# tohtsky/myFM

Hardware: AMD Instinct MI355X
Metric: Gibbs iterations/sec (rank=32) (higher is better)
Workload: dtype f64

## Files before the change

myfm_amd/csrc/mfm_res.hpp:

```cpp
#pragma once
#include <algorithm>
#include <cstdlib>
#include <cstring>
#include <atomic>
#include <string>
#include <thread>
#include <vector>

#include "mfm_common.hpp"
#include "mfm_mf_kernels.hpp"

namespace mfm {

#ifndef MFM_RES_CH
#define MFM_RES_CH 4
#endif
constexpr int RES_MAX_PEERS = 8;

struct ResArgs {
  double2 *eq;
  const double *e_in;
  double *e_slots;
  const int32_t *perm;
  const uint32_t *uidw;
// ... 48 lines not shown
  __hip_atomic_store(p + 1, b, __ATOMIC_RELAXED, __HIP_MEMORY_SCOPE_AGENT);
}

enum { RES_BAR_START = 0, RES_BAR_TOP = 16, RES_BAR_XCNT = 32, RES_BAR_GEN = 160, RES_BAR_CENSUS = 288, RES_BAR_WORDS = 416 };
struct ResBar {
  int xcc;
  unsigned long long n_x, nx;
};

__device__ __forceinline__ bool res_spin(const ResArgs &a, const unsigned long long *w, unsigned long long target, bool &dead) {
  unsigned spins = 0;
  while (__hip_atomic_load(w, __ATOMIC_RELAXED, __HIP_MEMORY_SCOPE_AGENT) < target) {
#ifndef MFM_RES_NO_SLEEP
    __builtin_amdgcn_s_sleep(1);
#endif
    if ((++spins & 1023u) == 0u) {
      if (spins > (1u << 22) || __hip_atomic_load(a.error, __ATOMIC_RELAXED, __HIP_MEMORY_SCOPE_AGENT) != 0) {
        __hip_atomic_store(a.error, 1, __ATOMIC_RELAXED, __HIP_MEMORY_SCOPE_AGENT);
        dead = true;
        return false;
      }
    }
  }
  return true;
}

__device__ __forceinline__ bool res_spin_sys(const ResArgs &a, const unsigned long long *w, unsigned long long target, bool &dead) {
  unsigned spins = 0;
  while (__hip_atomic_load(w, __ATOMIC_RELAXED, __HIP_MEMORY_SCOPE_SYSTEM) < target) {
    __builtin_amdgcn_s_sleep(2);
    if ((++spins & 1023u) == 0u) {
      const int seen = __hip_atomic_load(a.error, __ATOMIC_RELAXED, __HIP_MEMORY_SCOPE_AGENT);
      if (spins > (1u << 23) || seen != 0) {
        if (seen == 0) __hip_atomic_store(a.error, 2, __ATOMIC_RELAXED, __HIP_MEMORY_SCOPE_AGENT);
        dead = true;
        return false;
      }
    }
  }
  return true;
}

__device__ __forceinline__ void res_bar_init(const ResArgs &a, ResBar &rb, bool &dead) {
  unsigned x;
  asm volatile("s_getreg_b32 %0, hwreg(HW_REG_XCC_ID, 0, 4)" : "=s"(x));
  rb.xcc = (int)(x & 7u);
  __hip_atomic_fetch_add(a.bar + RES_BAR_CENSUS + 16 * rb.xcc, 1ull, __ATOMIC_RELAXED, __HIP_MEMORY_SCOPE_AGENT);
  asm volatile("s_waitcnt vmcnt(0)" ::: "memory");
  __hip_atomic_fetch_add(a.bar + RES_BAR_START, 1ull, __ATOMIC_RELAXED, __HIP_MEMORY_SCOPE_AGENT);
  rb.n_x = 1;
  rb.nx = 1;
  if (!res_spin(a, a.bar + RES_BAR_START, (unsigned long long)a.n_wg, dead)) return;
  rb.nx = 0;
  for (int i = 0; i < 8; i++) {
    const unsigned long long c = __hip_atomic_load(a.bar + RES_BAR_CENSUS + 16 * i, __ATOMIC_RELAXED, __HIP_MEMORY_SCOPE_AGENT);
    rb.nx += c > 0 ? 1 : 0;
    if (i == rb.xcc) rb.n_x = c;
  }
}

__device__ __forceinline__ void res_grid_barrier(const ResArgs &a, const ResBar &rb, unsigned long long k, int tid, bool &dead) {
  asm volatile("s_waitcnt vmcnt(0)" ::: "memory");
  __syncthreads();
  if (tid == 0 && !dead) {
    const unsigned long long old =
        __hip_atomic_fetch_add(a.bar + RES_BAR_XCNT + 16 * rb.xcc, 1ull, __ATOMIC_RELAXED, __HIP_MEMORY_SCOPE_AGENT);
    if (old + 1 == k * rb.n_x) {
      __builtin_amdgcn_fence(__ATOMIC_RELEASE, "agent");
      asm volatile("s_waitcnt vmcnt(0)" ::: "memory");
      __hip_atomic_fetch_add(a.bar + RES_BAR_TOP, 1ull, __ATOMIC_RELAXED, __HIP_MEMORY_SCOPE_AGENT);
      if (res_spin(a, a.bar + RES_BAR_TOP, k * rb.nx, dead))
        __hip_atomic_store(a.bar + RES_BAR_GEN + 16 * rb.xcc, k, __ATOMIC_RELAXED, __HIP_MEMORY_SCOPE_AGENT);
    } else {
      res_spin(a, a.bar + RES_BAR_GEN + 16 * rb.xcc, k, dead);
    }
    __builtin_amdgcn_fence(__ATOMIC_ACQUIRE, "agent");
  }
  __syncthreads();
}

typedef double res_d16_t __attribute__((ext_vector_type(16)));
typedef unsigned res_u4_t __attribute__((ext_vector_type(4)));

template <int NT, int NGV, int NGL, bool XCH = false, bool OVF = false>
__global__ __launch_bounds__(NT) void k_mf_resident(ResArgs a) {
  extern __shared__ __attribute__((aligned(16))) char res_smem[];
  constexpr int NW = NT / WAVE, NG = NGV + NGL, R = 16 * NG, RL = 16 * NGL;
  constexpr int B = 4;
  const int g = (int)blockIdx.x, tid = threadIdx.x, lane = tid & 63;
  const int wv = __builtin_amdgcn_readfirstlane(tid >> 6);
  const int U = a.umax;
  const double alpha_k = a.scal ? a.scal[0] : a.alpha, e_shift_k = a.scal ? a.scal[2] : a.e_shift;
  const int ngx = OVF ? a.ngx : 0, NGt = NG + ngx, Rt = 16 * NGt;
  d2_t *utab = (d2_t *)res_smem;
  double *elds = (double *)(utab + U);
  double *acc1 = elds + (size_t)RL * NT;
  double *acc2 = acc1 + NW * U;
  d2_t *wcarry = (d2_t *)(acc2 + NW * U);
  int *wflag = (int *)(wcarry + NW);
  const int32_t *perm_g = a.perm + (int64_t)g * Rt * NT;
  const int u0 = a.wg_user_ptr[g], nu = a.wg_user_ptr[g + 1] - u0;
  const int rb0 = a.wg_run_ptr[g];
  const int pad_item = a.n_items;
  const unsigned rb0b = 4u * (unsigned)rb0, padb = 16u * (unsigned)pad_item;
  const char *run_item_b = (const char *)a.run_item, *dv_b = (const char *)a.dv;
  double *acc1w = acc1 + wv * U, *acc2w = acc2 + wv * U;
  bool dead = false;
  unsigned long long nbar = 0;
  ResBar rbar;
  rbar.xcc = 0;
  rbar.n_x = rbar.nx = 1;
#define RES_STAMP0(k) \
  if (a.prof && tid == 0) a.prof[(int64_t)g * a.n_sw * 64 + 56 + (k)] = __builtin_amdgcn_s_memrealtime()
  RES_STAMP0(0);
  if (tid == 0) res_bar_init(a, rbar, dead);
  RES_STAMP0(1);
  const int wv_hi = wv >> 2;
#define RES_PRIO(j)                  \
  if ((((j) & 1) ^ wv_hi) != 0)      \
    __builtin_amdgcn_s_setprio(1);   \
  else                               \
    __builtin_amdgcn_s_setprio(0)
  const int trash_run = a.wg_run_ptr[g] + a.wg_nruns[g];
#define RES_STAMP(k)                                                                                      \
  if (a.prof && tid == 0) a.prof[((int64_t)g * a.n_sw + (f - f_first)) * 64 + (k)] = __builtin_amdgcn_s_memrealtime()

  for (int i = tid; i < 2 * NW * U; i += NT) acc1[i] = 0.0;
  for (int i = tid; i < U; i += NT) utab[i] = d2_t{0.0, 0.0};

  res_u4_t uw[NG];
  unsigned ux[NG];
  unsigned hbv[NG], nbv[NG];
#pragma unroll
  for (int j = 0; j < NG; j++) {
#pragma unroll
    for (int w = 0; w < 4; w++) uw[j][w] = a.uidw[((int64_t)g * (5 * NGt) + 5 * j + w) * NT + tid];
    ux[j] = a.uidw[((int64_t)g * (5 * NGt) + 5 * j + 4) * NT + tid];
    hbv[j] = a.headw[((int64_t)g * NGt + j) * NT + tid];
    nbv[j] = hbv[j] | (j == 0 ? 1u : 0u);
  }
  const unsigned nbx0 = OVF && ngx > 0 ? a.headw[((int64_t)g * NGt + NG) * NT + tid] : 0u;
  double *eog = OVF ? a.e_slots + ((int64_t)g * Rt + 16 * NG) * NT + tid : nullptr;
  const uint32_t *uidw_x = a.uidw + ((int64_t)g * (5 * NGt) + 5 * NG) * NT + tid;
  const uint32_t *headw_x = a.headw + ((int64_t)g * NGt + NG) * NT + tid;
  const int run0 = a.first_run[g * NT + tid];
  const bool head0 = (hbv[0] & 1u) != 0u;
#define RES_NIB(j, q) ((((nbv[j]) | ((j) + 1 < NG ? nbv[(j) + 1 < NG ? (j) + 1 : (j)] << 16 : nbx0 << 16)) >> (4 * (q))) & 15u)
#define RES_UIDS(j, bb, uid)                                                     \
  {                                                                              \
    const unsigned lo_ = uw[j][bb];                                              \
    uid[0] = (int)(lo_ & 0x3ffu);                                                \
    uid[1] = (int)((lo_ >> 10) & 0x3ffu);                                        \
    uid[2] = (int)((lo_ >> 20) & 0x3ffu);                                        \
    uid[3] = (int)((lo_ >> 30) | (((ux[j] >> (8 * (bb))) & 0xffu) << 2));        \
  }

#define RES_UIDSX(bb, uid)                                                       \
  {                                                                              \
    const unsigned lo_ = uwx[bb];                                                \
    uid[0] = (int)(lo_ & 0x3ffu);                                                \
    uid[1] = (int)((lo_ >> 10) & 0x3ffu);                                        \
    uid[2] = (int)((lo_ >> 20) & 0x3ffu);                                        \
    uid[3] = (int)((lo_ >> 30) | (((uxx >> (8 * (bb))) & 0xffu) << 2));          \
  }

#define RES_OPAQUE()                                                                            \
  _Pragma("unroll") for (int j_ = 0; j_ < NG; j_++) {                                           \
    asm volatile("" : "+v"(uw[j_]), "+v"(ux[j_]), "+v"(hbv[j_]), "+v"(nbv[j_]));                \
  }
  res_d16_t ev[NGV > 0 ? NGV : 1];
#pragma unroll
  for (int j = 0; j < NG; j++) {
#pragma unroll 1
    for (int bb = 0; bb < 4; bb++) {
      int row[B];
#pragma unroll
      for (int k = 0; k < B; k++) row[k] = a.e_in ? 0 : perm_g[(16 * j + 4 * bb + k) * NT + tid];
#pragma unroll
      for (int k = 0; k < B; k++) {
        const double x = (a.e_in ? a.e_in[((int64_t)g * Rt + 16 * j + 4 * bb + k) * NT + tid] : a.eq[row[k] < 0 ? 0 : row[k]].x) + e_shift_k;
        if (j < NGV)
          ev[j < NGV ? j : 0][4 * bb + k] = x;
        else
          elds[(16 * (j - NGV) + 4 * bb + k) * NT + tid] = x;
      }
    }
  }
  if (OVF) {
    for (int jx = 0; jx < ngx; jx++) {
#pragma unroll 4
      for (int i = 0; i < 16; i++) {
        const int64_t sl = 16 * (NG + jx) + i;
        const int row = a.e_in ? 0 : perm_g[sl * NT + tid];
        const double x = (a.e_in ? a.e_in[((int64_t)g * Rt + sl) * NT + tid] : a.eq[row < 0 ? 0 : row].x) + e_shift_k;
        eog[(16 * jx + i) * NT] = x;
      }
    }
  }
  __syncthreads();

  RES_STAMP0(2);
  const int f_first = a.f_begin - a.linear;
  for (int f = f_first; f < a.f_end; f++) {
    const bool lin = f < a.f_begin;
    double *Vf = lin ? a.w : a.V + (int64_t)f * a.D;
    const double *zf = lin ? a.zw : a.z + (int64_t)(f - a.f_begin) * a.D;
    const double *lamf = lin ? a.lam_w : a.lam + (int64_t)f * a.n_groups;
    const double *muf = lin ? a.mu_w : a.mu + (int64_t)f * a.n_groups;
    int uj = 0;
    double uold = 0.0, uz = 0.0, ulam = 0.0, umu = 0.0;
    if (tid < nu) {
      const int2 d = a.user_desc[u0 + tid];
      uj = d.x;
      uold = Vf[uj];
      uz = zf[uj];
      ulam = lamf[d.y];
      umu = muf[d.y];
    }
    RES_STAMP(0);
    {
      RES_OPAQUE();
      asm volatile(";; res sweep A");
      unsigned rcb = 4u * (unsigned)(run0 - 1);
      int itA[B];
      d2_t ddA[B];
      {
        int it0[B];
        const unsigned n0 = RES_NIB(0, 0), n1 = RES_NIB(0, 1);
#pragma unroll
        for (int k = 0; k < B; k++) {
          rcb += ((n0 >> k) & 1u) << 2;
          it0[k] = *(const int *)(run_item_b + ((n0 >> k) & 1u ? rcb : rb0b));
        }
#pragma unroll
        for (int k = 0; k < B; k++) {
          rcb += ((n1 >> k) & 1u) << 2;
          itA[k] = *(const int *)(run_item_b + ((n1 >> k) & 1u ? rcb : rb0b));
        }
#pragma unroll
        for (int k = 0; k < B; k++) ddA[k] = *(const d2_t *)(dv_b + ((n0 >> k) & 1u ? (unsigned)it0[k] << 4 : padb));
      }
      d2_t ddc = d2_t{0.0, 0.0};
      int itB[B];
      d2_t ddB[B];
#define RES_STEP_A(j, bb, iti, ito, ddi, ddo)                                                                              \
  {                                                                                                                        \
    const unsigned n4 = RES_NIB(j, bb), n4a = RES_NIB(j, (bb) + 1), n4b = RES_NIB(j, (bb) + 2);                            \
    _Pragma("unroll") for (int k = 0; k < B; k++) {                                                                        \
      rcb += ((n4b >> k) & 1u) << 2;                                                                                       \
      ito[k] = *(const int *)(run_item_b + ((n4b >> k) & 1u ? rcb : rb0b));                                                \
    }                                                                                                                      \
// ... 25 lines not shown
    const unsigned n4 = ((nbw >> (4 * (bb))) & 15u), n4a = ((nbw >> (4 * ((bb) + 1))) & 15u), n4b = ((nbw >> (4 * ((bb) + 2))) & 15u);                            \
    _Pragma("unroll") for (int k = 0; k < B; k++) {                                                                        \
      rcb += ((n4b >> k) & 1u) << 2;                                                                                       \
      ito[k] = *(const int *)(run_item_b + ((n4b >> k) & 1u ? rcb : rb0b));                                                \
    }                                                                                                                      \
    _Pragma("unroll") for (int k = 0; k < B; k++)                                                                          \
      ddo[k] = *(const d2_t *)(dv_b + ((n4a >> k) & 1u ? (unsigned)iti[k] << 4 : padb));                                   \
    int uid[B];                                                                                                            \
    RES_UIDSX(bb, uid);                                                                                                      \
    double up[B], ex[B];                                                                                                   \
    _Pragma("unroll") for (int k = 0; k < B; k++) {                                                                        \
      up[k] = utab[uid[k]][0];                                                                                             \
      ex[k] = eo[4 * (bb) + k];              \
    }                                                                                                                      \
    _Pragma("unroll") for (int k = 0; k < B; k++) {                                                                        \
      const bool need = ((n4 >> k) & 1u) != 0u;                                                                            \
      ddc[0] = need ? ddi[k][0] : ddc[0];                                                                                  \
      ddc[1] = need ? ddi[k][1] : ddc[1];                                                                                  \
      const double er = ex[k] + up[k] * ddc[0];                                                                            \
      eo[4 * (bb) + k] = er;                                                             \
      const double c = ddc[1];                                                                                             \
      __hip_atomic_fetch_add(&acc1w[uid[k]], (-er) * c, __ATOMIC_RELAXED, __HIP_MEMORY_SCOPE_WORKGROUP);                   \
      __hip_atomic_fetch_add(&acc2w[uid[k]], c * c, __ATOMIC_RELAXED, __HIP_MEMORY_SCOPE_WORKGROUP);                       \
    }                                                                                                                      \
  }
#pragma unroll
      for (int j = 0; j < NG; j++) {
        RES_PRIO(j);
#pragma unroll
        for (int bp = 0; bp < 2; bp++) {
          RES_STEP_A(j, 2 * bp, itA, itB, ddA, ddB);
          RES_STEP_A(j, 2 * bp + 1, itB, itA, ddB, ddA);
        }
      }
      asm volatile(";; res sweep end");
      if (OVF) {
        unsigned hb_c = nbx0;
        for (int jx = 0; jx < ngx; jx++) {
          res_u4_t uwx;
#pragma unroll
          for (int w = 0; w < 4; w++) uwx[w] = uidw_x[(5 * jx + w) * NT];
          const unsigned uxx = uidw_x[(5 * jx + 4) * NT];
          const unsigned hb_n = jx + 1 < ngx ? headw_x[(jx + 1) * NT] : 0u;
          const unsigned nbw = hb_c | (hb_n << 16);
          res_d16_t eo;
#pragma unroll
          for (int i = 0; i < 16; i++) eo[i] = eog[(16 * jx + i) * NT];
#pragma unroll 1
          for (int bp = 0; bp < 2; bp++) {
            RES_STEP_AX(2 * bp, itA, itB, ddA, ddB);
            RES_STEP_AX(2 * bp + 1, itB, itA, ddB, ddA);
          }
#pragma unroll
          for (int i = 0; i < 16; i++) eog[(16 * jx + i) * NT] = eo[i];
          hb_c = hb_n;
        }
      }
#undef RES_STEP_A
#undef RES_STEP_AX
    }
    __syncthreads();
    RES_STAMP(1);
    if (tid < nu) {
      double S1 = 0.0, S2 = 0.0;
#pragma unroll
      for (int w = 0; w < NW; w++) {
        S1 += acc1[w * U + tid];
        S2 += acc2[w * U + tid];
        acc1[w * U + tid] = 0.0;
        acc2[w * U + tid] = 0.0;
      }
      const double fresh = PMainV::draw(S1, S2, uold, alpha_k, ulam, umu, uz);
      Vf[uj] = fresh;
      if (XCH && a.xmodel) {
        for (int r = 0; r < a.xworld; r++)
          if (r != a.xrank)
            __hip_atomic_store((lin ? a.xw[r] : a.xV[r] + (int64_t)f * a.D) + uj, fresh, __ATOMIC_RELAXED, __HIP_MEMORY_SCOPE_SYSTEM);
      }
      utab[tid] = d2_t{lin ? 1.0 : fresh, fresh - uold};
    }
    __syncthreads();
    RES_STAMP(2);
    {
      bool have_head = false;
      double f1 = 0.0, f2 = 0.0, s1 = 0.0, s2 = 0.0;
      d2_t *part2 = (d2_t *)a.partials;
      char *part_b = (char *)a.partials - 16;
      const unsigned trashb = 16u * (unsigned)(trash_run + 1);
      {
        RES_OPAQUE();
        asm volatile(";; res sweep B");
        unsigned rcb = 4u * (unsigned)(run0 - 1);
        unsigned rcCb = 16u * (unsigned)(run0 - 1);
        int itA[B];
        double ccA[B];
        {
          int it0[B];
          const unsigned n0 = RES_NIB(0, 0), n1 = RES_NIB(0, 1);
#pragma unroll
          for (int k = 0; k < B; k++) {
            rcb += ((n0 >> k) & 1u) << 2;
            it0[k] = *(const int *)(run_item_b + ((n0 >> k) & 1u ? rcb : rb0b));
          }
#pragma unroll
          for (int k = 0; k < B; k++) {
            rcb += ((n1 >> k) & 1u) << 2;
            itA[k] = *(const int *)(run_item_b + ((n1 >> k) & 1u ? rcb : rb0b));
          }
#pragma unroll
          for (int k = 0; k < B; k++) ccA[k] = *(const double *)(dv_b + 8 + ((n0 >> k) & 1u ? (unsigned)it0[k] << 4 : padb));
        }
        double ccc = 0.0;
        int itB[B];
        double ccB[B];
#define RES_PARTIAL_STORE() *(d2_t *)(part_b + (head && have_head ? rcCb : trashb)) = d2_t{s1, s2}
#define RES_STEP_B(j, bb, iti, ito, cci, cco)                                                                              \
  {                                                                                                                        \
    const unsigned n4 = RES_NIB(j, bb), n4a = RES_NIB(j, (bb) + 1), n4b = RES_NIB(j, (bb) + 2);                            \
    const unsigned h4 = (hbv[j] >> (4 * (bb))) & 15u;                                                                      \
    _Pragma("unroll") for (int k = 0; k < B; k++) {                                                                        \
      rcb += ((n4b >> k) & 1u) << 2;                                                                                       \
      ito[k] = *(const int *)(run_item_b + ((n4b >> k) & 1u ? rcb : rb0b));                                                \
    }                                                                                                                      \
    _Pragma("unroll") for (int k = 0; k < B; k++)                                                                          \
      cco[k] = *(const double *)(dv_b + 8 + ((n4a >> k) & 1u ? (unsigned)iti[k] << 4 : padb));                             \
    int uid[B];                                                                                                            \
    RES_UIDS(j, bb, uid);                                                                                                  \
    d2_t ut[B];                                                                                                            \
    double ex[B];                                                                                                          \
    _Pragma("unroll") for (int k = 0; k < B; k++) {                                                                        \
      ut[k] = utab[uid[k]];                                                                                                \
      ex[k] = j < NGV ? ev[j < NGV ? j : 0][4 * (bb) + k] : elds[(16 * (j - NGV) + 4 * (bb) + k) * NT + tid];              \
    }                                                                                                                      \
    _Pragma("unroll") for (int k = 0; k < B; k++) {                                                                        \
      const bool need = ((n4 >> k) & 1u) != 0u;                                                                            \
      const bool head = ((h4 >> k) & 1u) != 0u;                                                                            \
      ccc = need ? cci[k] : ccc;                                                                                           \
      rcCb += need ? 16u : 0u;                                                         \
                              \
      RES_PARTIAL_STORE();                                                                                                 \
      f1 = head && !have_head ? s1 : f1;                                                                                   \
      f2 = head && !have_head ? s2 : f2;                                                                                   \
      have_head = have_head || head;                                                                                       \
      const double er = ex[k] + ccc * ut[k][1];                                                                            \
      if (j < NGV)                                                                                                         \
        ev[j < NGV ? j : 0][4 * (bb) + k] = er;                                                                            \
      else                                                                                                                 \
        elds[(16 * (j - NGV) + 4 * (bb) + k) * NT + tid] = er;                                                             \
      s1 = (head ? 0.0 : s1) + (-er) * ut[k][0];                                                                           \
      s2 = (head ? 0.0 : s2) + ut[k][0] * ut[k][0];                                                                        \
    }                                                                                                                      \
  }
#define RES_STEP_BX(bb, iti, ito, cci, cco)                                                                                 \
  {                                                                                                                        \
    const unsigned n4 = ((nbw >> (4 * (bb))) & 15u), n4a = ((nbw >> (4 * ((bb) + 1))) & 15u), n4b = ((nbw >> (4 * ((bb) + 2))) & 15u);                            \
    const unsigned h4 = (hb_c >> (4 * (bb))) & 15u;                                                                       \
    _Pragma("unroll") for (int k = 0; k < B; k++) {                                                                        \
      rcb += ((n4b >> k) & 1u) << 2;                                                                                       \
      ito[k] = *(const int *)(run_item_b + ((n4b >> k) & 1u ? rcb : rb0b));                                                \
    }                                                                                                                      \
    _Pragma("unroll") for (int k = 0; k < B; k++)                                                                          \
      cco[k] = *(const double *)(dv_b + 8 + ((n4a >> k) & 1u ? (unsigned)iti[k] << 4 : padb));                             \
    int uid[B];                                                                                                            \
    RES_UIDSX(bb, uid);                                                                                                      \
    d2_t ut[B];                                                                                                            \
    double ex[B];                                                                                                          \
    _Pragma("unroll") for (int k = 0; k < B; k++) {                                                                        \
      ut[k] = utab[uid[k]];                                                                                                \
      ex[k] = eo[4 * (bb) + k];              \
    }                                                                                                                      \
    _Pragma("unroll") for (int k = 0; k < B; k++) {                                                                        \
      const bool need = ((n4 >> k) & 1u) != 0u;                                                                            \
      const bool head = ((h4 >> k) & 1u) != 0u;                                                                            \
      ccc = need ? cci[k] : ccc;                                                                                           \
      rcCb += need ? 16u : 0u;                                                         \
                              \
      RES_PARTIAL_STORE();                                                                                                 \
      f1 = head && !have_head ? s1 : f1;                                                                                   \
      f2 = head && !have_head ? s2 : f2;                                                                                   \
      have_head = have_head || head;                                                                                       \
      const double er = ex[k] + ccc * ut[k][1];                                                                            \
      eo[4 * (bb) + k] = er;                                                             \
      s1 = (head ? 0.0 : s1) + (-er) * ut[k][0];                                                                           \
      s2 = (head ? 0.0 : s2) + ut[k][0] * ut[k][0];                                                                        \
    }                                                                                                                      \
  }
#pragma unroll
        for (int j = 0; j < NG; j++) {
          RES_PRIO(j);
#pragma unroll 1
          for (int bp = 0; bp < 2; bp++) {
            RES_STEP_B(j, 2 * bp, itA, itB, ccA, ccB);
            RES_STEP_B(j, 2 * bp + 1, itB, itA, ccB, ccA);
          }
          if (a.prof && lane == 0 && (wv == 4 || wv == 7))
            a.prof[((int64_t)g * a.n_sw + (f - f_first)) * 64 + 16 + (wv == 4 ? 0 : 20) + j] = __builtin_amdgcn_s_memrealtime();
        }
        asm volatile(";; res sweep end");
        if (OVF) {
          unsigned hb_c = nbx0;
          for (int jx = 0; jx < ngx; jx++) {
            res_u4_t uwx;
#pragma unroll
            for (int w = 0; w < 4; w++) uwx[w] = uidw_x[(5 * jx + w) * NT];
            const unsigned uxx = uidw_x[(5 * jx + 4) * NT];
            const unsigned hb_n = jx + 1 < ngx ? headw_x[(jx + 1) * NT] : 0u;
            const unsigned nbw = hb_c | (hb_n << 16);
            res_d16_t eo;
#pragma unroll
            for (int i = 0; i < 16; i++) eo[i] = eog[(16 * jx + i) * NT];
#pragma unroll 1
            for (int bp = 0; bp < 2; bp++) {
              RES_STEP_BX(2 * bp, itA, itB, ccA, ccB);
              RES_STEP_BX(2 * bp + 1, itB, itA, ccB, ccA);
            }
#pragma unroll
            for (int i = 0; i < 16; i++) eog[(16 * jx + i) * NT] = eo[i];
            hb_c = hb_n;
          }
        }
#undef RES_STEP_B
#undef RES_STEP_BX
#undef RES_PARTIAL_STORE
      }
      if (a.prof && lane == 0)
        a.prof[((int64_t)g * a.n_sw + (f - f_first)) * 64 + 8 + wv] = __builtin_amdgcn_s_memrealtime();
      double v1 = s1, v2 = s2;
      int fl = have_head ? 1 : 0;
      wave_segscan2(v1, v2, fl);
      if (lane == 63) {
        wcarry[wv] = d2_t{v1, v2};
        wflag[wv] = fl;
      }
      double x1 = dpp_f64<0x138, 0xf>(v1), x2 = dpp_f64<0x138, 0xf>(v2);
      int xf = dpp_i32<0x138, 0xf>(fl, 0);
      if (lane == 0) {
        x1 = 0.0;
        x2 = 0.0;
        xf = 0;
      }
      lds_barrier();
      if (have_head && tid > 0) {
        if (!xf) {
          double c1 = 0.0, c2 = 0.0;
          for (int w = 0; w < wv; w++) {
            const d2_t cw = wcarry[w];
            const bool fw = wflag[w] != 0;
            c1 = (fw ? 0.0 : c1) + cw[0];
            c2 = (fw ? 0.0 : c2) + cw[1];
          }
          x1 = c1 + x1;
          x2 = c2 + x2;
        }
        const int closing = head0 ? run0 - 1 : run0;
        part2[closing] = d2_t{x1 + f1, x2 + f2};
      }
    }
    RES_STAMP(3);
    constexpr int CH = MFM_RES_CH;
    const int c0 = a.ent_ptr[g] >> 6, c1 = a.ent_ptr[g + 1] >> 6;
    const int per = (c1 - c0 + NW - 1) / NW;
    const int wb = c0 + wv * per, we = wb + per < c1 ? wb + per : c1;
    const int i0 = a.wg_item_ptr[g], ni = a.wg_item_ptr[g + 1] - i0;
    const bool more = f + 1 < a.f_end;
    int ij = 0;
    double iold = 0.0, iz = 0.0, ivn = 0.0, ilam = 0.0, imu = 0.0;
    if (tid < ni) {
      const int2 d = a.item_desc[i0 + tid];
      ij = d.x;
      iold = Vf[ij];
      iz = zf[ij];
      ivn = more ? a.V[(int64_t)(f + 1) * a.D + ij] : 0.0;
      ilam = lamf[d.y];
      imu = muf[d.y];
    }
    int2 en[CH];
#pragma unroll
    for (int k = 0; k < CH; k++) en[k] = make_int2(0, 0);
    if (wb < we) {
#pragma unroll
      for (int k = 0; k < CH; k++) en[k] = a.entries[(int64_t)(wb + k < we ? wb + k : wb) * WAVE + lane];
    }
    res_grid_barrier(a, rbar, ++nbar, tid, dead);
    RES_STAMP(4);
    {
      const d2_t *part2 = (const d2_t *)a.partials;
      for (int cb = wb; cb < we; cb += CH) {
        d2_t sv[CH];
#pragma unroll
        for (int k = 0; k < CH; k++) sv[k] = part2[en[k].x];
        int il[CH];
#pragma unroll
        for (int k = 0; k < CH; k++) il[k] = en[k].y;
        if (cb + CH < we) {
#pragma unroll
          for (int k = 0; k < CH; k++) en[k] = a.entries[(int64_t)(cb + CH + k < we ? cb + CH + k : cb + CH) * WAVE + lane];
        }
#pragma unroll
        for (int k = 0; k < CH; k++) {
          if (cb + k >= we) break;
          __hip_atomic_fetch_add(&acc1[wv * U + il[k]], sv[k][0], __ATOMIC_RELAXED, __HIP_MEMORY_SCOPE_WORKGROUP);
          __hip_atomic_fetch_add(&acc2[wv * U + il[k]], sv[k][1], __ATOMIC_RELAXED, __HIP_MEMORY_SCOPE_WORKGROUP);
        }
      }
      __syncthreads();
      double S1 = 0.0, S2 = 0.0;
      if (tid < ni) {
#pragma unroll
        for (int w = 0; w < NW; w++) {
          S1 += acc1[w * U + tid];
          S2 += acc2[w * U + tid];
          acc1[w * U + tid] = 0.0;
          acc2[w * U + tid] = 0.0;
        }
      }
      if (XCH) {
        const unsigned long long E = a.xepoch0 + (unsigned long long)(f - f_first) + 1ull;
        const int64_t stride = 2 * ((int64_t)a.n_items + 1), par = (int64_t)(E & 1ull);
        if (tid < ni) {
          const int64_t off = ((int64_t)a.xrank * 2 + par) * stride + 2 * (int64_t)(i0 + tid);
          for (int r = 0; r < a.xworld; r++) {
            __hip_atomic_store(a.xsum[r] + off, S1, __ATOMIC_RELAXED, __HIP_MEMORY_SCOPE_SYSTEM);
            __hip_atomic_store(a.xsum[r] + off + 1, S2, __ATOMIC_RELAXED, __HIP_MEMORY_SCOPE_SYSTEM);
          }
        }
        asm volatile("s_waitcnt vmcnt(0)" ::: "memory");
        __syncthreads();
        if (tid == 0 && !dead) {
          const unsigned long long old = __hip_atomic_fetch_add(a.xarrive, 1ull, __ATOMIC_RELAXED, __HIP_MEMORY_SCOPE_AGENT);
          if (old + 1 == (unsigned long long)a.n_wg * E) {
            for (int r = 0; r < a.xworld && !a.xch_break; r++)
              __hip_atomic_store(a.xflag[r] + 16 * a.xrank, E, __ATOMIC_RELEASE, __HIP_MEMORY_SCOPE_SYSTEM);
          }
          for (int r = 0; r < a.xworld && !dead; r++) res_spin_sys(a, a.xflag[a.xrank] + 16 * r, E, dead);
        }
        __syncthreads();
        if (tid < ni) {
          S1 = S2 = 0.0;
// ... 640 lines not shown
      }
    }
    std::vector<int2> h_entries((size_t)h_eptr[G], make_int2(zero_run, 0));
    {
      std::vector<int64_t> pos((size_t)G);
      for (int g = 0; g < G; g++) pos[g] = h_eptr[g];
      for (int g = 0; g < G; g++)
        for (size_t l = 0; l < wg_run_item[g].size(); l++) {
          const int32_t c = wg_run_item[g][l];
          const int sgl = slice_of[c];
          h_entries[(size_t)pos[sgl]++] = make_int2(run_base[g] + (int32_t)l, c - h_iptr[sgl]);
        }
    }
    if (h_entries.size() >= ((size_t)1 << 31)) return fail("too many entries");
    lds_bytes = (size_t)RL * NT * 8 + (size_t)2 * (NT / WAVE) * umax * 8 + (size_t)umax * 16 + (size_t)(NT / WAVE) * 16 + (NT / WAVE) * 4 + 64;
    if (lds_bytes > 160 * 1024 - 512) return fail("LDS");
    uidw.upload(h_uidw);
    headw.upload(h_headw);
    run_item.upload(h_run_item);
    perm.upload(h_perm);
    first_run.upload(h_first);
    wg_user_ptr.upload(h_uptr);
    user_desc.upload(h_udesc.data(), h_udesc.size());
    wg_item_ptr.upload(h_iptr);
    ent_ptr.upload(h_eptr);
    entries.upload(h_entries.data(), h_entries.size());
    wg_run_ptr.upload(run_base);
    wg_nruns.upload(nruns);
    e_slots.alloc((size_t)G * cap_slots);
    {
      std::vector<int32_t> h_run_feat(h_run_item.size() + 8, -1);
      for (size_t r = 0; r < h_run_item.size(); r++) h_run_feat[r] = h_run_item[r] < n_items ? items[(size_t)h_run_item[r]] : -1;
      run_feat.upload(h_run_feat);
      std::vector<int32_t> h_fill((size_t)G);
      for (int g = 0; g < G; g++) h_fill[g] = (int32_t)fill[g];
      wg_fill.upload(h_fill);
      sums.alloc((size_t)G);
      y_slots = DevBuf<double>();
    }
    h_nruns = nruns;
    if (env_flag("MFM_RES_PROF")) {
      h_diag.assign((size_t)G, "");
      for (int g = 0; g < G; g++) {
        int64_t maxlen = 0;
        for (int64_t u = ucut[g]; u < ucut[g + 1]; u++) maxlen = std::max(maxlen, ustart[u + 1] - ustart[u]);
        int64_t sinstr = 0, maxst = 0, nthr_head = 0;
        for (int w = 0; w < NT / WAVE; w++) {
          std::vector<char> hh(WAVE, 0);
          std::vector<int> st(WAVE, 0);
          for (int r = 0; r < R; r++) {
            bool any = false;
            for (int l = 0; l < WAVE; l++) {
              const int t = w * WAVE + l;
              const bool head = (h_headw[((size_t)g * HW + r / 16) * NT + t] >> (r % 16)) & 1u;
              if (head && hh[l]) {
                any = true;
                st[l]++;
              }
              hh[l] = hh[l] || head;
            }
            sinstr += any;
          }
          for (int l = 0; l < WAVE; l++) {
            maxst = std::max<int64_t>(maxst, st[l]);
            nthr_head += hh[l];
          }
        }
        char buf[160];
        std::snprintf(buf, sizeof buf, "users %d maxlen %lld rows %lld store-instr %lld max-stores/thread %lld threads-with-head %lld",
                      (int)(ucut[g + 1] - ucut[g]), (long long)maxlen, (long long)fill[g], (long long)sinstr, (long long)maxst,
                      (long long)nthr_head);
        h_diag[g] = buf;
      }
    }
    scols.upload(items);
    {
      std::vector<int2> h_idesc(items.size());
      for (size_t i = 0; i < items.size(); i++) {
        const int32_t j = items[i];
        h_idesc[i] = make_int2(j, group_of && (size_t)j < group_of->size() ? (*group_of)[j] : 0);
      }
      item_desc.upload(h_idesc.data(), h_idesc.size());
    }
    partials.alloc((size_t)2 * ((size_t)zero_run + 1));
    MFM_HIP_CHECK(hipMemset(partials.p, 0, (size_t)16 * ((size_t)zero_run + 1)));
    dv.alloc((size_t)2 * (n_items + 1));
    bar.alloc(RES_BAR_WORDS);
    ready = true;
    why.clear();
    return true;
  }
  bool fail(const char *w) {
    why = w;
    ready = false;
    return false;
  }
};

static inline hipError_t res_occupancy(const ResPlan &rp, int *per_cu) {
  *per_cu = 0;
  const void *fn = nullptr;
  if (rp.RV == 16 && rp.RL == 0)
    fn = (const void *)k_mf_resident<512, 1, 0>;
  else if (rp.RV == 32 && rp.RL == 0)
    fn = (const void *)k_mf_resident<512, 2, 0>;
  else if (rp.RV == 64 && rp.RL == 16)
    fn = rp.RX ? (const void *)k_mf_resident<512, 4, 1, false, true> : (const void *)k_mf_resident<512, 4, 1>;
  else
    return hipErrorInvalidValue;
  hipError_t e = hipFuncSetAttribute(fn, hipFuncAttributeMaxDynamicSharedMemorySize, 160 * 1024);
  if (e != hipSuccess) return e;
  return hipOccupancyMaxActiveBlocksPerMultiprocessor(per_cu, fn, 512, rp.lds_bytes);
}

static inline void run_sweep_resident(hipStream_t s, Timing &tm, ResPlan &rp, int kernel_class, double2 *eq, double *V, int64_t D,
                                      int f_begin, int f_end, const double *zbase, const double *lam, const double *mu,
                                      const int32_t *group, int n_groups, double alpha, int *error,
                                      double *w = nullptr, const double *zw = nullptr, const double *lam_w = nullptr,
                                      const double *mu_w = nullptr, double e_shift = 0.0, bool load_slots = false,
                                      bool no_store = false, const double *scal = nullptr) {
  ResArgs a;
  std::memset(&a, 0, sizeof(a));
  a.scal = scal;
  a.eq = eq;
  a.e_slots = rp.e_slots.p;
  a.ngx = rp.RX / 16;
  a.no_store = no_store ? 1 : 0;
  a.e_in = load_slots ? rp.e_slots.p : nullptr;
  a.linear = w ? 1 : 0;
  a.n_sw = f_end - f_begin + a.linear;
  a.w = w;
  a.zw = zw;
  a.lam_w = lam_w;
  a.mu_w = mu_w;
  a.e_shift = e_shift;
  a.perm = rp.perm.p;
  a.uidw = rp.uidw.p;
  a.headw = rp.headw.p;
  a.run_item = rp.run_item.p;
  a.first_run = rp.first_run.p;
  a.wg_user_ptr = rp.wg_user_ptr.p;
  a.user_desc = rp.user_desc.p;
  a.wg_item_ptr = rp.wg_item_ptr.p;
  a.ent_ptr = rp.ent_ptr.p;
  a.entries = rp.entries.p;
  a.wg_run_ptr = rp.wg_run_ptr.p;
  a.wg_nruns = rp.wg_nruns.p;
  a.scols = rp.scols.p;
  a.item_desc = rp.item_desc.p;
  a.partials = rp.partials.p;
  a.dv = rp.dv.p;
  a.V = V;
  a.D = D;
  a.f_begin = f_begin;
  a.f_end = f_end;
  a.z = zbase;
  a.lam = lam;
  a.mu = mu;
  a.group = group;
  a.n_groups = n_groups;
  a.alpha = alpha;
  a.n_items = rp.n_items;
  a.umax = rp.umax;
  a.bar = rp.bar.p;
  a.n_wg = rp.G;
  a.error = error;
  const bool xch = rp.xworld > 1;
  a.xch_break = xch && rp.xrank == 1 && env_flag("MFM_RES_XCH_BREAK");
  a.xworld = rp.xworld;
  a.xrank = rp.xrank;
  a.xepoch0 = rp.xepoch;
  a.xarrive = rp.xarrive.p;
  a.xmodel = xch && rp.peers_model ? 1 : 0;
  for (int r = 0; r < RES_MAX_PEERS; r++) {
    a.xsum[r] = rp.peer_sum[r];
    a.xflag[r] = rp.peer_flag[r];
    a.xw[r] = rp.peer_w[r];
    a.xV[r] = rp.peer_V[r];
  }
  if (xch && !rp.peers_set) throw Error(MFM_ERR_RUNTIME, "row-sharded persistent sweep: the peers' exchange buffers are not set (mfm_peer_set)");
  static int prof_launch = 0;
  const bool prof = env_flag("MFM_RES_PROF") && ++prof_launch == env_int("MFM_RES_PROF", 0);
  DevBuf<unsigned long long> prof_buf;
  if (prof) {
    prof_buf.alloc((size_t)rp.G * a.n_sw * 64);
    MFM_HIP_CHECK(hipMemsetAsync(prof_buf.p, 0, (size_t)rp.G * a.n_sw * 512, s));
    a.prof = prof_buf.p;
  }
  const int K = a.n_sw;
  double bytes = (8.0 + (load_slots ? 0.0 : 4.0) + 1.4 + (no_store ? 0.0 : 8.0)) * rp.n_rows + K * 48.0 * rp.n_runs;
  if (rp.RX) bytes += (double)K * (16.0 + 1.75) * (double)rp.G * rp.NT * rp.RX;
  hipLaunchKernelGGL(k_res_init_dv, dim3((rp.n_items + 256) / 256), dim3(256), 0, s,
                     w ? (const double *)nullptr : V + (int64_t)f_begin * D, rp.scols.p, rp.n_items,
                     rp.dv.p, rp.bar.p);
  TimedLaunch t(tm, s, kernel_class, bytes);
#define MFM_RES_LAUNCH(RV_, RL_)                                                                                              \
  do {                                                                                                                        \
    static DeviceOnce raised;                                                                                                 \
    if (raised.need()) {                                                                                                      \
      MFM_HIP_CHECK(hipFuncSetAttribute((const void *)k_mf_resident<512, RV_ / 16, RL_ / 16>,                                  \
                                        hipFuncAttributeMaxDynamicSharedMemorySize, 160 * 1024));                             \
      raised.mark();                                                                                                          \
    }                                                                                                                         \
    if (xch) {                                                                                                                \
      static DeviceOnce raised_x;                                                                                             \
      if (raised_x.need()) {                                                                                                  \
        MFM_HIP_CHECK(hipFuncSetAttribute((const void *)k_mf_resident<512, RV_ / 16, RL_ / 16, true>,                          \
                                          hipFuncAttributeMaxDynamicSharedMemorySize, 160 * 1024));                           \
        raised_x.mark();                                                                                                      \
      }                                                                                                                       \
      hipLaunchKernelGGL((k_mf_resident<512, RV_ / 16, RL_ / 16, true>), dim3(rp.G), dim3(512), rp.lds_bytes, s, a);            \
    } else {                                                                                                                  \
      hipLaunchKernelGGL((k_mf_resident<512, RV_ / 16, RL_ / 16>), dim3(rp.G), dim3(512), rp.lds_bytes, s, a);                  \
    }                                                                                                                         \
  } while (0)
  if (rp.RV == 16 && rp.RL == 0)
    MFM_RES_LAUNCH(16, 0);
  else if (rp.RV == 32 && rp.RL == 0)
    MFM_RES_LAUNCH(32, 0);
  else if (rp.RV == 64 && rp.RL == 16 && rp.RX > 0) {
    if (xch) throw Error(MFM_ERR_RUNTIME, "internal: no row-sharded resident kernel with overflow slots");
    static DeviceOnce raised_o;
    if (raised_o.need()) {
      MFM_HIP_CHECK(hipFuncSetAttribute((const void *)k_mf_resident<512, 4, 1, false, true>, hipFuncAttributeMaxDynamicSharedMemorySize, 160 * 1024));
      raised_o.mark();
    }
    hipLaunchKernelGGL((k_mf_resident<512, 4, 1, false, true>), dim3(rp.G), dim3(512), rp.lds_bytes, s, a);
  } else if (rp.RV == 64 && rp.RL == 16)
    MFM_RES_LAUNCH(64, 16);
  else
    throw Error(MFM_ERR_RUNTIME, "internal: no resident kernel variant for this plan");
#undef MFM_RES_LAUNCH
  MFM_HIP_CHECK(hipGetLastError());
// ... 189 lines not shown
```

myfm_amd/csrc/mfm_res_plan.hpp:

```cpp
#pragma once
#include <chrono>

#include <hipcub/hipcub.hpp>

#include "mfm_res.hpp"

namespace mfm {

namespace rp {

constexpr int TB = 256;

__global__ void k_rows(const int32_t *__restrict__ colidx, int64_t N, int32_t *__restrict__ bflag, int32_t *__restrict__ ucnt,
                       int32_t *__restrict__ icnt, int32_t *__restrict__ red) {
  const int64_t r = (int64_t)blockIdx.x * blockDim.x + threadIdx.x;
  int32_t mu = -1, mi = 0x7fffffff;
  if (r < N) {
    const int2 c = ((const int2 *)colidx)[r];
    const bool b = r == 0 || c.x != colidx[2 * (r - 1)];
    bflag[r] = b ? 1 : 0;
    if (b) atomicAdd(&ucnt[c.x], 1);
    atomicAdd(&icnt[c.y], 1);
    mu = c.x;
    mi = c.y;
// ... 376 lines not shown
  for (int g = 0; g < G; g++) nruns[g] = h_hrun0[g + 1] - h_hrun0[g];
  const int64_t counter = h_hrun0[G];
  rpn.n_runs = counter;
  if (counter >= ((int64_t)1 << 31) - 2) return rpn.fail("too many runs");
  const std::vector<int32_t> run_base = ResPlan::run_bases(nruns);
  const int32_t zero_run = run_base[G];
  rpn.wg_run_ptr.upload(run_base);
  rpn.wg_nruns.upload(nruns);
  rpn.run_item.alloc((size_t)zero_run + 1);
  hipLaunchKernelGGL(k_fill32, grid(zero_run + 1), dim3(TB), 0, s, rpn.run_item.p, (int64_t)zero_run + 1, n_items);
  DevBuf<int32_t> run_item_c, runs_per_item;
  run_item_c.alloc((size_t)std::max<int64_t>(counter, 1));
  runs_per_item.alloc_zero((size_t)n_items, s);
  hipLaunchKernelGGL(k_runs, grid(N), dim3(TB), 0, s, key2.p, headf.p, hs.p, hrun0.p, rpn.wg_run_ptr.p, rpn.item_bits, N, run_item_c.p,
                     rpn.run_item.p, runs_per_item.p);
  rpn.first_run.alloc((size_t)G * NT);
  hipLaunchKernelGGL(k_first, grid((int64_t)G * NT), dim3(TB), 0, s, hs.p, rowcut.p, hrun0.p, rpn.wg_run_ptr.p, G, R, NT, rpn.first_run.p);
  lap("slots, heads, runs, first");
  std::vector<int32_t> h_slot_ptr((size_t)n_items + 1, 0), h_iptr;
  {
    const std::vector<int32_t> rpi = download(runs_per_item.p, (size_t)n_items, s);
    for (int c = 0; c < n_items; c++) h_slot_ptr[(size_t)c + 1] = h_slot_ptr[c] + rpi[c];
  }
  if (!rpn.choose_item_slices(h_slot_ptr, counter, h_iptr)) return false;
  int imax = 0;
  for (int g = 0; g < G; g++) imax = std::max(imax, h_iptr[g + 1] - h_iptr[g]);
  rpn.umax = std::max(maxu, imax) + 1;
  if (rpn.umax > 1024) return rpn.fail("internal: user field");
  const int UW = 5 * (R / 16), HW = R / 16;
  rpn.uidw.alloc((size_t)G * UW * NT);
  rpn.headw.alloc((size_t)G * HW * NT);
  hipLaunchKernelGGL(k_pack, grid((int64_t)G * HW * NT), dim3(TB), 0, s, uid.p, headf.p, rowcut.p, G, R, NT, rpn.umax, rpn.uidw.p, rpn.headw.p);
  std::vector<int32_t> h_eptr((size_t)G + 1, 0), h_sstart((size_t)G + 1, 0);
  for (int g = 0; g < G; g++) {
    const int64_t cnt = h_slot_ptr[h_iptr[g + 1]] - h_slot_ptr[h_iptr[g]];
    const int64_t e = h_eptr[g] + ((cnt + WAVE - 1) / WAVE) * WAVE;
    if (e >= ((int64_t)1 << 31)) return rpn.fail("too many entries");
    h_eptr[g + 1] = (int32_t)e;
    h_sstart[g + 1] = h_sstart[g] + (int32_t)cnt;
  }
  rpn.wg_item_ptr.upload(h_iptr);
  rpn.ent_ptr.upload(h_eptr);
  rpn.entries.alloc((size_t)h_eptr[G]);
  if (h_eptr[G]) hipLaunchKernelGGL(k_fill_int2, grid(h_eptr[G]), dim3(TB), 0, s, rpn.entries.p, (int64_t)h_eptr[G], make_int2(zero_run, 0));
  if (counter > 0) {
    DevBuf<int32_t> sstart;
    sstart.upload(h_sstart);
    DevBuf<uint32_t> sk, sk2;
    DevBuf<int32_t> sv, sv2;
    sk.alloc((size_t)counter);
    sk2.alloc((size_t)counter);
    sv.alloc((size_t)counter);
    sv2.alloc((size_t)counter);
    hipLaunchKernelGGL(k_slice_keys, grid(counter), dim3(TB), 0, s, run_item_c.p, rpn.wg_item_ptr.p, G, counter, sk.p, sv.p);
    sort_pairs(sk, sk2, sv, sv2, counter, gbits, tmp, s);
    hipLaunchKernelGGL(k_entries, grid(counter), dim3(TB), 0, s, sk2.p, sv2.p, run_item_c.p, hrun0.p, rpn.wg_run_ptr.p, rpn.wg_item_ptr.p,
                       rpn.ent_ptr.p, sstart.p, G, counter, rpn.entries.p);
    MFM_HIP_CHECK(hipStreamSynchronize(s));
  }
  lap("slices, pack, entries");
  DevBuf<int32_t> d_group;
  if (group_of && (int64_t)group_of->size() >= D0) d_group.upload(group_of->data(), (size_t)D0);
  rpn.user_desc.alloc((size_t)h_uptr[G]);
  hipLaunchKernelGGL(k_user_desc, grid((int64_t)n_users + n_emp), dim3(TB), 0, s, d_users.p, empties.p, d_ucut.p, rpn.wg_user_ptr.p, d_group.p, G,
                     n_users, n_emp, rpn.user_desc.p);
  rpn.item_desc.alloc((size_t)n_items);
  hipLaunchKernelGGL(k_item_desc, grid(n_items), dim3(TB), 0, s, rpn.scols.p, d_group.p, n_items, rpn.item_desc.p);
  rpn.run_feat.alloc((size_t)zero_run + 1 + 8);
  hipLaunchKernelGGL(k_run_feat, grid((int64_t)zero_run + 9), dim3(TB), 0, s, rpn.run_item.p, rpn.scols.p, n_items, (int64_t)zero_run + 1,
                     (int64_t)zero_run + 9, rpn.run_feat.p);
  {
    std::vector<int32_t> h_fill((size_t)G);
    for (int g = 0; g < G; g++) h_fill[g] = h_rowcut[g + 1] - h_rowcut[g];
    rpn.wg_fill.upload(h_fill);
  }
  rpn.lds_bytes = (size_t)rpn.RL * NT * 8 + (size_t)2 * (NT / WAVE) * rpn.umax * 8 + (size_t)rpn.umax * 16 + (size_t)(NT / WAVE) * 16 +
                  (NT / WAVE) * 4 + 64;
  if (rpn.lds_bytes > 160 * 1024 - 512) return rpn.fail("LDS");
  rpn.e_slots.alloc((size_t)G * cap_slots);
  rpn.sums.alloc((size_t)G);
  rpn.y_slots = DevBuf<double>();
  rpn.h_nruns = nruns;
  rpn.h_diag.clear();
  rpn.partials.alloc((size_t)2 * ((size_t)zero_run + 1));
  MFM_HIP_CHECK(hipMemsetAsync(rpn.partials.p, 0, (size_t)16 * ((size_t)zero_run + 1), s));
  rpn.dv.alloc((size_t)2 * (n_items + 1));
  rpn.bar.alloc(RES_BAR_WORDS);
  MFM_HIP_CHECK(hipStreamSynchronize(s));
  MFM_HIP_CHECK(hipGetLastError());
  lap("descriptors, buffers");
  rpn.ready = true;
  rpn.why.clear();
  return true;
}

static inline std::string res_plan_compare(const ResPlan &a, const ResPlan &b, hipStream_t s) {
  if (a.G != b.G || a.RV != b.RV || a.RL != b.RL || a.RX != b.RX || a.umax != b.umax || a.item_bits != b.item_bits || a.n_items != b.n_items ||
      a.n_rows != b.n_rows || a.n_runs != b.n_runs || a.lds_bytes != b.lds_bytes)
    return "scalars";
  auto same = [&](const void *p, size_t np, const void *q, size_t nq, size_t elem) {
    if (np != nq) return false;
    std::vector<char> x(np * elem), y(nq * elem);
    if (np) {
      MFM_HIP_CHECK(hipMemcpyAsync(x.data(), p, np * elem, hipMemcpyDeviceToHost, s));
      MFM_HIP_CHECK(hipMemcpyAsync(y.data(), q, nq * elem, hipMemcpyDeviceToHost, s));
    }
    MFM_HIP_CHECK(hipStreamSynchronize(s));
    return x == y;
  };
#define MFM_RP_CMP(f) \
  if (!same(a.f.p, a.f.n, b.f.p, b.f.n, sizeof(*a.f.p))) return #f;
  MFM_RP_CMP(perm)
  MFM_RP_CMP(first_run)
  MFM_RP_CMP(wg_run_ptr)
  MFM_RP_CMP(wg_nruns)
  MFM_RP_CMP(wg_user_ptr)
  MFM_RP_CMP(wg_item_ptr)
  MFM_RP_CMP(ent_ptr)
  MFM_RP_CMP(scols)
  MFM_RP_CMP(entries)
  MFM_RP_CMP(uidw)
  MFM_RP_CMP(headw)
  MFM_RP_CMP(run_item)
  MFM_RP_CMP(user_desc)
  MFM_RP_CMP(item_desc)
  MFM_RP_CMP(run_feat)
  MFM_RP_CMP(wg_fill)
#undef MFM_RP_CMP
  return "";
}

}
```

Measured before the change: 348.4.

## Cut sweep-B register pressure: drop nbv, reload first-head partial, swap halves

Removes the duplicated nbv register array and derives its value from hbv instead. It also drops the per-step tracking of the first head's partial (f1/f2/have_head). That value is now read back from the global partials buffer after the sweep, which adds a vmcnt wait and a shifted partials base with one extra slot. It rotates the ev/uw/ux register halves with v_swap so both unrolled steps use fixed static indices. The aim is to lower VGPR pressure and per-element select work in the hot sweep, at the cost of an extra global load and a memory wait.

```diff
diff --git a/myfm_amd/csrc/mfm_res.hpp b/myfm_amd/csrc/mfm_res.hpp
--- a/myfm_amd/csrc/mfm_res.hpp
+++ b/myfm_amd/csrc/mfm_res.hpp
@@ -154,6 +154,15 @@
 typedef double res_d16_t __attribute__((ext_vector_type(16)));
 typedef unsigned res_u4_t __attribute__((ext_vector_type(4)));
 
+__device__ __forceinline__ void res_swap(double &a, double &b) {
+  unsigned al = (unsigned)__double2loint(a), ah = (unsigned)__double2hiint(a);
+  unsigned bl = (unsigned)__double2loint(b), bh = (unsigned)__double2hiint(b);
+  asm("v_swap_b32 %0, %1" : "+v"(al), "+v"(bl));
+  asm("v_swap_b32 %0, %1" : "+v"(ah), "+v"(bh));
+  a = __hiloint2double((int)ah, (int)al);
+  b = __hiloint2double((int)bh, (int)bl);
+}
+
 template <int NT, int NGV, int NGL, bool XCH = false, bool OVF = false>
 __global__ __launch_bounds__(NT) void k_mf_resident(ResArgs a) {
   extern __shared__ __attribute__((aligned(16))) char res_smem[];
@@ -202,14 +211,13 @@
 
   res_u4_t uw[NG];
   unsigned ux[NG];
-  unsigned hbv[NG], nbv[NG];
+  unsigned hbv[NG];
 #pragma unroll
   for (int j = 0; j < NG; j++) {
 #pragma unroll
     for (int w = 0; w < 4; w++) uw[j][w] = a.uidw[((int64_t)g * (5 * NGt) + 5 * j + w) * NT + tid];
     ux[j] = a.uidw[((int64_t)g * (5 * NGt) + 5 * j + 4) * NT + tid];
     hbv[j] = a.headw[((int64_t)g * NGt + j) * NT + tid];
-    nbv[j] = hbv[j] | (j == 0 ? 1u : 0u);
   }
   const unsigned nbx0 = OVF && ngx > 0 ? a.headw[((int64_t)g * NGt + NG) * NT + tid] : 0u;
   double *eog = OVF ? a.e_slots + ((int64_t)g * Rt + 16 * NG) * NT + tid : nullptr;
@@ -217,7 +225,8 @@
   const uint32_t *headw_x = a.headw + ((int64_t)g * NGt + NG) * NT + tid;
   const int run0 = a.first_run[g * NT + tid];
   const bool head0 = (hbv[0] & 1u) != 0u;
-#define RES_NIB(j, q) ((((nbv[j]) | ((j) + 1 < NG ? nbv[(j) + 1 < NG ? (j) + 1 : (j)] << 16 : nbx0 << 16)) >> (4 * (q))) & 15u)
+#define RES_NBV(j) ((j) == 0 ? hbv[0] | 1u : hbv[j])
+#define RES_NIB(j, q) ((((RES_NBV(j)) | ((j) + 1 < NG ? hbv[(j) + 1 < NG ? (j) + 1 : (j)] << 16 : nbx0 << 16)) >> (4 * (q))) & 15u)
 #define RES_UIDS(j, bb, uid)                                                     \
   {                                                                              \
     const unsigned lo_ = uw[j][bb];                                              \
@@ -238,7 +247,7 @@
 
 #define RES_OPAQUE()                                                                            \
   _Pragma("unroll") for (int j_ = 0; j_ < NG; j_++) {                                           \
-    asm volatile("" : "+v"(uw[j_]), "+v"(ux[j_]), "+v"(hbv[j_]), "+v"(nbv[j_]));                \
+    asm volatile("" : "+v"(uw[j_]), "+v"(ux[j_]), "+v"(hbv[j_]));                                \
   }
   res_d16_t ev[NGV > 0 ? NGV : 1];
 #pragma unroll
@@ -430,9 +439,8 @@
     __syncthreads();
     RES_STAMP(2);
     {
-      bool have_head = false;
+      unsigned hall = 0u;
       double f1 = 0.0, f2 = 0.0, s1 = 0.0, s2 = 0.0;
-      d2_t *part2 = (d2_t *)a.partials;
       char *part_b = (char *)a.partials - 16;
       const unsigned trashb = 16u * (unsigned)(trash_run + 1);
       {
@@ -461,8 +469,8 @@
         double ccc = 0.0;
         int itB[B];
         double ccB[B];
-#define RES_PARTIAL_STORE() *(d2_t *)(part_b + (head && have_head ? rcCb : trashb)) = d2_t{s1, s2}
-#define RES_STEP_B(j, bb, iti, ito, cci, cco)                                                                              \
+#define RES_PARTIAL_STORE() *(d2_t *)(part_b + (head ? rcCb : trashb)) = d2_t{s1, s2}
+#define RES_STEP_B(j, bb, sb, iti, ito, cci, cco)                                                                              \
   {                                                                                                                        \
     const unsigned n4 = RES_NIB(j, bb), n4a = RES_NIB(j, (bb) + 1), n4b = RES_NIB(j, (bb) + 2);                            \
     const unsigned h4 = (hbv[j] >> (4 * (bb))) & 15u;                                                                      \
@@ -473,12 +481,12 @@
     _Pragma("unroll") for (int k = 0; k < B; k++)                                                                          \
       cco[k] = *(const double *)(dv_b + 8 + ((n4a >> k) & 1u ? (unsigned)iti[k] << 4 : padb));                             \
     int uid[B];                                                                                                            \
-    RES_UIDS(j, bb, uid);                                                                                                  \
+    RES_UIDS(j, sb, uid);                                                                                                  \
     d2_t ut[B];                                                                                                            \
     double ex[B];                                                                                                          \
     _Pragma("unroll") for (int k = 0; k < B; k++) {                                                                        \
       ut[k] = utab[uid[k]];                                                                                                \
-      ex[k] = j < NGV ? ev[j < NGV ? j : 0][4 * (bb) + k] : elds[(16 * (j - NGV) + 4 * (bb) + k) * NT + tid];              \
+      ex[k] = j < NGV ? ev[j < NGV ? j : 0][4 * (sb) + k] : elds[(16 * (j - NGV) + 4 * (bb) + k) * NT + tid];              \
     }                                                                                                                      \
     _Pragma("unroll") for (int k = 0; k < B; k++) {                                                                        \
       const bool need = ((n4 >> k) & 1u) != 0u;                                                                            \
@@ -487,12 +495,9 @@
       rcCb += need ? 16u : 0u;                                                         \
                               \
       RES_PARTIAL_STORE();                                                                                                 \
-      f1 = head && !have_head ? s1 : f1;                                                                                   \
-      f2 = head && !have_head ? s2 : f2;                                                                                   \
-      have_head = have_head || head;                                                                                       \
       const double er = ex[k] + ccc * ut[k][1];                                                                            \
       if (j < NGV)                                                                                                         \
-        ev[j < NGV ? j : 0][4 * (bb) + k] = er;                                                                            \
+        ev[j < NGV ? j : 0][4 * (sb) + k] = er;                                                                            \
       else                                                                                                                 \
         elds[(16 * (j - NGV) + 4 * (bb) + k) * NT + tid] = er;                                                             \
       s1 = (head ? 0.0 : s1) + (-er) * ut[k][0];                                                                           \
@@ -524,9 +529,6 @@
       rcCb += need ? 16u : 0u;                                                         \
                               \
       RES_PARTIAL_STORE();                                                                                                 \
-      f1 = head && !have_head ? s1 : f1;                                                                                   \
-      f2 = head && !have_head ? s2 : f2;                                                                                   \
-      have_head = have_head || head;                                                                                       \
       const double er = ex[k] + ccc * ut[k][1];                                                                            \
       eo[4 * (bb) + k] = er;                                                             \
       s1 = (head ? 0.0 : s1) + (-er) * ut[k][0];                                                                           \
@@ -538,13 +540,33 @@
           RES_PRIO(j);
 #pragma unroll 1
           for (int bp = 0; bp < 2; bp++) {
-            RES_STEP_B(j, 2 * bp, itA, itB, ccA, ccB);
-            RES_STEP_B(j, 2 * bp + 1, itB, itA, ccB, ccA);
+            RES_STEP_B(j, 2 * bp, 0, itA, itB, ccA, ccB);
+            RES_STEP_B(j, 2 * bp + 1, 1, itB, itA, ccB, ccA);
+            if (j < NGV) {
+              res_d16_t &v_ = ev[j < NGV ? j : 0];
+#pragma unroll
+              for (int i = 0; i < 8; i++) {
+                double lo_ = v_[i], hi_ = v_[i + 8];
+                res_swap(lo_, hi_);
+                v_[i] = lo_;
+                v_[i + 8] = hi_;
+              }
+            }
+#pragma unroll
+            for (int i = 0; i < 2; i++) {
+              unsigned lo_ = uw[j][i], hi_ = uw[j][i + 2];
+              asm("v_swap_b32 %0, %1" : "+v"(lo_), "+v"(hi_));
+              uw[j][i] = lo_;
+              uw[j][i + 2] = hi_;
+            }
+            ux[j] = (ux[j] >> 16) | (ux[j] << 16);
           }
           if (a.prof && lane == 0 && (wv == 4 || wv == 7))
             a.prof[((int64_t)g * a.n_sw + (f - f_first)) * 64 + 16 + (wv == 4 ? 0 : 20) + j] = __builtin_amdgcn_s_memrealtime();
         }
         asm volatile(";; res sweep end");
+#pragma unroll
+        for (int j = 0; j < NG; j++) hall |= hbv[j];
         if (OVF) {
           unsigned hb_c = nbx0;
           for (int jx = 0; jx < ngx; jx++) {
@@ -554,6 +576,7 @@
             const unsigned uxx = uidw_x[(5 * jx + 4) * NT];
             const unsigned hb_n = jx + 1 < ngx ? headw_x[(jx + 1) * NT] : 0u;
             const unsigned nbw = hb_c | (hb_n << 16);
+            hall |= hb_c;
             res_d16_t eo;
 #pragma unroll
             for (int i = 0; i < 16; i++) eo[i] = eog[(16 * jx + i) * NT];
@@ -573,6 +596,14 @@
       }
       if (a.prof && lane == 0)
         a.prof[((int64_t)g * a.n_sw + (f - f_first)) * 64 + 8 + wv] = __builtin_amdgcn_s_memrealtime();
+      const bool have_head = hall != 0u;
+      unsigned closeb = 16u * (unsigned)run0 + (head0 ? 0u : 16u);
+      asm volatile("" : "+v"(closeb));
+      asm volatile("s_waitcnt vmcnt(0)" ::: "memory");
+      if (have_head && tid > 0) {
+        f1 = __hip_atomic_load((const double *)(part_b + closeb), __ATOMIC_RELAXED, __HIP_MEMORY_SCOPE_AGENT);
+        f2 = __hip_atomic_load((const double *)(part_b + closeb) + 1, __ATOMIC_RELAXED, __HIP_MEMORY_SCOPE_AGENT);
+      }
       double v1 = s1, v2 = s2;
       int fl = have_head ? 1 : 0;
       wave_segscan2(v1, v2, fl);
@@ -600,8 +631,7 @@
           x1 = c1 + x1;
           x2 = c2 + x2;
         }
-        const int closing = head0 ? run0 - 1 : run0;
-        part2[closing] = d2_t{x1 + f1, x2 + f2};
+        *(d2_t *)(part_b + closeb) = d2_t{x1 + f1, x2 + f2};
       }
     }
     RES_STAMP(3);
@@ -1408,8 +1438,8 @@
       }
       item_desc.upload(h_idesc.data(), h_idesc.size());
     }
-    partials.alloc((size_t)2 * ((size_t)zero_run + 1));
-    MFM_HIP_CHECK(hipMemset(partials.p, 0, (size_t)16 * ((size_t)zero_run + 1)));
+    partials.alloc((size_t)2 * ((size_t)zero_run + 2));
+    MFM_HIP_CHECK(hipMemset(partials.p, 0, (size_t)16 * ((size_t)zero_run + 2)));
     dv.alloc((size_t)2 * (n_items + 1));
     bar.alloc(RES_BAR_WORDS);
     ready = true;
@@ -1474,7 +1504,7 @@
   a.wg_nruns = rp.wg_nruns.p;
   a.scols = rp.scols.p;
   a.item_desc = rp.item_desc.p;
-  a.partials = rp.partials.p;
+  a.partials = rp.partials.p + 2;
   a.dv = rp.dv.p;
   a.V = V;
   a.D = D;
diff --git a/myfm_amd/csrc/mfm_res_plan.hpp b/myfm_amd/csrc/mfm_res_plan.hpp
--- a/myfm_amd/csrc/mfm_res_plan.hpp
+++ b/myfm_amd/csrc/mfm_res_plan.hpp
@@ -482,8 +482,8 @@
   rpn.y_slots = DevBuf<double>();
   rpn.h_nruns = nruns;
   rpn.h_diag.clear();
-  rpn.partials.alloc((size_t)2 * ((size_t)zero_run + 1));
-  MFM_HIP_CHECK(hipMemsetAsync(rpn.partials.p, 0, (size_t)16 * ((size_t)zero_run + 1), s));
+  rpn.partials.alloc((size_t)2 * ((size_t)zero_run + 2));
+  MFM_HIP_CHECK(hipMemsetAsync(rpn.partials.p, 0, (size_t)16 * ((size_t)zero_run + 2), s));
   rpn.dv.alloc((size_t)2 * (n_items + 1));
   rpn.bar.alloc(RES_BAR_WORDS);
   MFM_HIP_CHECK(hipStreamSynchronize(s));
```

After: 346.3. About the same (-0.6%).
